# zombie-einstein/bourse

Hardware: NVIDIA B200
Metric: orders_per_sec (higher is better)
Workload: dtype u32

## Files before the change

### bourse_b200/csrc/book.cuh

```cuda
#pragma once
#include <cstdint>

namespace bb {

typedef uint32_t u32;
typedef uint64_t u64;

#define BB_NIL 0xFFFFFFFFu
#define BB_TAG_FREE 0xFFFFFFFFu
#define BB_FULL 0xFFFFFFFFu

enum { ST_NEW = 0, ST_ACTIVE = 1, ST_FILLED = 2, ST_CANCELLED = 3, ST_REJECTED = 4 };
#define META_STATUS_MASK 7u
#define META_BID 8u
#define META_GHOST 16u

#define ERR_CAP_ORDERS 0x01u
#define ERR_CAP_TRADES 0x02u
#define ERR_CAP_PAGES 0x04u
#define ERR_CAP_QUEUE 0x08u
#define ERR_BAD_ID 0x10u
#define ERR_GRANULE 0x20u
#define ERR_CAP_STEPS 0x40u
#define ERR_CAP_LIVE 0x80u
// ... 65 lines not shown
    u32 v;
    asm volatile("ld.global.u32 %0, [%1];" : "=r"(v) : "l"(a));
    return v;
}
__device__ __forceinline__ u64 ldg64(u64 a) {
    u64 v;
    asm volatile("ld.global.u64 %0, [%1];" : "=l"(v) : "l"(a));
    return v;
}
__device__ __forceinline__ uint4 ldg128(u64 a) {
    uint4 v;
    asm volatile("ld.global.v4.u32 {%0,%1,%2,%3}, [%4];" : "=r"(v.x), "=r"(v.y), "=r"(v.z), "=r"(v.w) : "l"(a));
    return v;
}
__device__ __forceinline__ void stg32(u64 a, u32 v) { asm volatile("st.global.u32 [%0], %1;" ::"l"(a), "r"(v) : "memory"); }
__device__ __forceinline__ void stg64(u64 a, u64 v) { asm volatile("st.global.u64 [%0], %1;" ::"l"(a), "l"(v) : "memory"); }
__device__ __forceinline__ void stg128(u64 a, u32 x, u32 y, u32 z, u32 w) {
    asm volatile("st.global.v4.u32 [%0], {%1,%2,%3,%4};" ::"l"(a), "r"(x), "r"(y), "r"(z), "r"(w) : "memory");
}

__device__ __forceinline__ void prefetch_l2(u64 a) { asm volatile("prefetch.global.L2 [%0];" ::"l"(a)); }

#define OH_PRICE 0u
#define OH_VOL 4u
#define OH_NEXT 8u
#define OH_PREV 12u
#define OH_KEYT 16u
#define OH_META 24u
#define OH_SVOL 28u
#define OC_ARR 32u
#define OC_END 40u
#define OC_TRADER 48u
#define PG_VC 0u
#define PG_HT 256u
#define PG_VOL(l) (8u * (l))
#define PG_CNT(l) (8u * (l) + 4u)
#define PG_HEAD(l) (256u + 8u * (l))
#define PG_TAIL(l) (260u + 8u * (l))

#define FL_TRADING 1u
#define FL_HAS_ASK 2u
#define FL_HAS_BID 4u

struct Geo {
    u32 p_total, p_smem, granule, tick, max_orders, max_trades;
    u64 tr_base;
    u64 blobs_base;
    u64 blob_stride;
    u32 d_win_lo, d_levels, d_live;
    u32 pc_off;
};
template <u32 LP_, u32 NWMAX_> struct DenseLayout;
#define ENG_PAGED 0
#define ENG_FAST 1
#define ENG_DENSE 2
#define ENG_DENSE_L 3
#define ENG_PAGED_RES 4
#define ENG_DEEP 5
template <int ENG_> struct GeoT : Geo {
    static constexpr bool FAST = ENG_ == ENG_FAST;
    static constexpr bool RES = ENG_ == ENG_FAST || ENG_ == ENG_PAGED_RES;
    static constexpr bool DENSE = ENG_ == ENG_DENSE || ENG_ == ENG_DENSE_L;
    typedef DenseLayout<(ENG_ == ENG_DENSE_L ? 256u : 128u), (ENG_ == ENG_DENSE_L ? 32u : 8u)> DL;
};
template <class G> __device__ __forceinline__ u32 ptot(const G& g) { return G::FAST ? 32u : g.p_total; }
template <class G> __device__ __forceinline__ u32 gran(const G& g) { return G::FAST ? 1u : g.granule; }

struct Book {
    u64 t, max_key_time;
    u32 n_orders, n_trades, trade_vol;
    u32 vol_ask, vol_bid;
    u32 bq_ask, bq_bid;
    u32 flags, err;
    u32 d_instr, d_trans, d_volume;
    u32 sb;
    u32 tag_lane;
    u64 oh;
    u32 env;
    u64 blob;
    u32 lane;
    u32 free_top;
    u32 ags;
    u64 tr_ptr;
};

__device__ __forceinline__ u32 tag_addr(const Book& b, u32 i) { return b.sb + 128u + 4u * i; }
template <class G> __device__ __forceinline__ u32 vmap_addr(const G& g, const Book& b, u32 i) { return b.sb + 128u + 4u * (ptot(g) + i); }
template <class G> __device__ __forceinline__ u32 qmap_addr(const G& g, const Book& b, u32 i) { return b.sb + 128u + 4u * (2u * ptot(g) + i); }

struct PageS {
    u32 a;
};
struct PageG {
    u64 a;
};
__device__ __forceinline__ u32 pld(PageS p, u32 off) { return lds(p.a + off); }
__device__ __forceinline__ u32 pld(PageG p, u32 off) { return ldg32(p.a + off); }
__device__ __forceinline__ void pst(PageS p, u32 off, u32 v) { sts(p.a + off, v); }
__device__ __forceinline__ void pst(PageG p, u32 off, u32 v) { stg32(p.a + off, v); }
__device__ __forceinline__ uint2 pld2(PageS p, u32 off) {
    const u64 v = lds64(p.a + off);
    return make_uint2((u32)v, (u32)(v >> 32));
}
__device__ __forceinline__ uint2 pld2(PageG p, u32 off) {
    const u64 v = ldg64(p.a + off);
    return make_uint2((u32)v, (u32)(v >> 32));
}
__device__ __forceinline__ void pst2(PageS p, u32 off, u32 x, u32 y) { sts64(p.a + off, ((u64)y << 32) | x); }
__device__ __forceinline__ void pst2(PageG p, u32 off, u32 x, u32 y) { stg64(p.a + off, ((u64)y << 32) | x); }

template <class G> __device__ __forceinline__ u32 page_off(const G& g, u32 slot) { return 128u + 12u * ptot(g) + slot * 512u; }
template <class G> __device__ __forceinline__ PageS page_s(const G& g, const Book& b, u32 slot) {
    return PageS{b.sb + page_off(g, slot)};
}
template <class G> __device__ __forceinline__ PageG page_g(const G& g, const Book& b, u32 slot) {
    return PageG{b.blob + page_off(g, slot)};
}
template <class G> __device__ __forceinline__ uint2 level_pair_any(const G& g, const Book& b, u32 slot, u32 l) {
    return (G::RES || slot < g.p_smem) ? pld2(page_s(g, b, slot), PG_VC + 8u * l) : pld2(page_g(g, b, slot), PG_VC + 8u * l);
}

__device__ __forceinline__ bool has_best(const Book& b, u32 side) { return (b.flags >> (1u + side)) & 1u; }
__device__ __forceinline__ u32 best_q(const Book& b, u32 side) { return side ? b.bq_bid : b.bq_ask; }
__device__ __forceinline__ void set_best(Book& b, u32 side, u32 q) {
    if (side) b.bq_bid = q; else b.bq_ask = q;
    b.flags |= FL_HAS_ASK << side;
}
__device__ __forceinline__ void add_side_vol(Book& b, u32 side, u32 dv) {
    if (side) b.vol_bid += dv; else b.vol_ask += dv;
}

template <class G> __device__ __forceinline__ bool to_level(const G& g, u32 price, u32* q) {
    if (G::FAST || gran(g) == 1u) {
        *q = price;
        return true;
    }
    const u32 x = price / gran(g);
    *q = x;
    return x * gran(g) == price;
}

#define PCACHE_ENTRIES 128u
template <class G> __device__ __forceinline__ u32 find_page(const G& g, const Book& b, u32 side, u32 pkey) {
    const u32 want = (pkey << 1) | side;
    u32 ca = 0;
    if constexpr (!G::FAST) {
        ca = b.sb + g.pc_off + (want & (PCACHE_ENTRIES - 1u));
        const u32 s = lds8(ca);
        if (lds(tag_addr(b, s)) == want) return s;
    }
    for (u32 base = 0; base < ptot(g); base += 32) {
        const u32 m = __ballot_sync(BB_FULL, lds(b.tag_lane + 4u * base) == want);
        if (m) {
            const u32 slot = base + __ffs(m) - 1;
            if constexpr (!G::FAST) sts8(ca, slot);
            return slot;
        }
    }
    return BB_NIL;
}

template <class G> __device__ __forceinline__ u32 alloc_page(const G& g, Book& b, u32 side, u32 pkey) {
    for (u32 base = 0; base < ptot(g); base += 32) {
        const bool usable = !G::RES || (base + b.lane) < g.p_smem;
        const u32 m = __ballot_sync(BB_FULL, usable && lds(b.tag_lane + 4u * base) == BB_TAG_FREE);
        if (m) {
// ... 538 lines not shown
```

### bourse_b200/csrc/dense.cuh

```cuda
#pragma once

namespace bb {

#define D_NIL 0xFFu

template <u32 LP_, u32 NWMAX_> struct DenseLayout {
    static constexpr u32 LP = LP_, NWMAX = NWMAX_;
    static constexpr u32 OFF_ID = 128u, OFF_SV = OFF_ID + 4u * LP, OFF_SL = OFF_SV + 4u * LP, OFF_FS = OFF_SL + 4u * LP;
    static constexpr u32 OFF_BM = OFF_FS + LP, OFF_LV = OFF_BM + 8u * NWMAX;
    static constexpr u32 image_bytes(u32 W) { return OFF_LV + 16u * W; }
};
typedef DenseLayout<128u, 8u> DenseSmall;
typedef DenseLayout<256u, 32u> DenseLarge;

__device__ __forceinline__ void stg128_cs(u64 a, u32 x, u32 y, u32 z, u32 w) {
    asm volatile("st.global.cs.v4.u32 [%0], {%1,%2,%3,%4};" ::"l"(a), "r"(x), "r"(y), "r"(z), "r"(w) : "memory");
}
__device__ __forceinline__ void stg64v(u64 a, u32 x, u32 y) { asm volatile("st.global.v2.u32 [%0], {%1,%2};" ::"l"(a), "r"(x), "r"(y) : "memory"); }

template <class G> __device__ __forceinline__ u32 d_lv(const Book& b, u32 side, u32 q) { return b.sb + G::DL::OFF_LV + 16u * q + 8u * side; }
template <class G> __device__ __forceinline__ u32 d_bm(const Book& b, u32 side, u32 w) {
    return b.sb + G::DL::OFF_BM + 4u * (side ? G::DL::NWMAX : 0u) + 4u * w;
}

template <class G> __device__ __forceinline__ void d_next_best(Book& b, u32 side, u32 q, u32 m) {
    u32 w = q >> 5;
    if (side == 0u) {
        while (m == 0u) {
            if (++w >= G::DL::NWMAX) {
                b.flags &= ~FL_HAS_ASK;
                return;
            }
            m = lds(d_bm<G>(b, 0u, w));
        }
        b.bq_ask = (w << 5) + (u32)__ffs(m) - 1u;
    } else {
        while (m == 0u) {
            if (w == 0u) {
                b.flags &= ~FL_HAS_BID;
                return;
            }
            --w;
            m = lds(d_bm<G>(b, 1u, w));
        }
        b.bq_bid = (w << 5) + 31u - (u32)__clz(m);
    }
}

template <class G> __device__ __forceinline__ void d_log_trade(const G& g, Book& b, u64 t, u32 passive_bid, u32 price, u32 vol,
                                                               u32 active, u32 passive) {
    if (b.n_trades < g.max_trades) {
        stg128_cs(b.tr_ptr, (u32)t, (u32)(t >> 32), price, vol);
        stg128_cs(b.tr_ptr + 16u, active, passive, passive_bid, 0u);
        b.tr_ptr += 32u;
    } else if (g.max_trades) {
        b.err |= ERR_CAP_TRADES;
    }
    b.n_trades += 1;
}

template <class G> __device__ __forceinline__ void d_free_slot(Book& b, u32 slot) {
    sts(b.sb + 4u * slot + G::DL::OFF_ID, BB_NIL);
    sts8(b.sb + G::DL::OFF_FS + b.free_top, slot);
    b.free_top += 1;
}

template <bool STEPPED, class G> __device__ __forceinline__ u32 d_match(const G& g, Book& b, u32 side, u32 price, u32 vol, u32 id, u64 t) {
    const u32 o = side ^ 1u;
    while (vol > 0u && has_best(b, o)) {
        const u32 bq = best_q(b, o);
        const u32 bprice = g.d_win_lo + bq;
        if (side ? (price < bprice) : (price > bprice)) break;
        const u32 la = d_lv<G>(b, o, bq);
        const u64 lv = lds64(la);
        const u32 lvol = (u32)lv, hi = (u32)(lv >> 32);
        const u32 head = (hi >> 16) & 0xFFu;
        const u32 sa = b.sb + 4u * head;
        const u32 pid = lds(sa + G::DL::OFF_ID), pvol = lds(sa + G::DL::OFF_SV);
        const u32 tv = min(vol, pvol);
        vol -= tv;
        d_log_trade(g, b, t, o, bprice, tv, id, pid);
        b.trade_vol += tv;
        if (!STEPPED) {
            b.d_volume += tv;
            b.d_trans += 1;
        }
        add_side_vol(b, o, 0u - tv);
        const u64 pa = b.oh + (u64)pid * ORD_STRIDE;
        if (pvol == tv) {
            stg32(pa + OH_VOL, 0u);
            stg32(pa + OH_META, ST_FILLED | (o ? META_BID : 0u));
            stg64(pa + OC_END, t);
            const u32 nxt = lds8(sa + G::DL::OFF_SL);
            d_free_slot<G>(b, head);
            if ((hi & 0xFFFFu) == 1u) {
                const u32 ba = d_bm<G>(b, o, bq >> 5);
                const u32 m = lds(ba) & ~(1u << (bq & 31u));
                sts(ba, m);
                d_next_best<G>(b, o, bq, m);
            } else {
                sts64(la, ((u64)((hi & 0xFF00FFFFu) - 1u + (nxt << 16)) << 32) | (u64)(lvol - tv));
            }
        } else {
            sts(sa + G::DL::OFF_SV, pvol - tv);
            stg32(pa + OH_VOL, pvol - tv);
            sts(la, lvol - tv);
        }
    }
    return vol;
}

template <bool CHECK_TIME, bool CHECK_SLOTS, class G> __device__ __forceinline__ u32 d_insert(const G& g, Book& b, u32 side, u32 price, u64 t,
                                                                            u32 id, u32 vol) {
    u32 q = price - g.d_win_lo;
    if (q >= g.d_levels) {
        b.err |= ERR_CAP_PAGES;
        q = 0u;
    }
    if (CHECK_SLOTS && b.free_top == 0u) {
        b.err |= ERR_CAP_LIVE;
        return 0u;
    }
    b.free_top -= 1;
    const u32 slot = lds8(b.sb + G::DL::OFF_FS + b.free_top);
    const u32 la = d_lv<G>(b, side, q);
    const u32 ba = d_bm<G>(b, side, q >> 5);
    const u32 bit = 1u << (q & 31u);
    const u32 bw = lds(ba);
    const u32 sa = b.sb + 4u * slot;
    u32 prev = D_NIL;
    if (bw & bit) {
        const u64 lv = lds64(la);
        const u32 hi = (u32)(lv >> 32);
        prev = hi >> 24;
        if (CHECK_TIME && t <= b.max_key_time) {
            const u32 tid = lds(b.sb + 4u * prev + G::DL::OFF_ID);
            if (t <= ldg64(b.oh + (u64)tid * ORD_STRIDE + OH_KEYT)) b.err |= ERR_TIME_ORDER;
        }
        sts64(la, ((u64)(((hi & 0x00FFFFFFu) + 1u) | (slot << 24)) << 32) | (u64)((u32)lv + vol));
        sts8(b.sb + 4u * prev + G::DL::OFF_SL, slot);
    } else {
        sts64(la, ((u64)(1u | (slot << 16) | (slot << 24)) << 32) | (u64)vol);
        sts(ba, bw | bit);
        const bool better = !has_best(b, side) || (side ? q > b.bq_bid : q < b.bq_ask);
        if (better) set_best(b, side, q);
    }
    sts(sa + G::DL::OFF_ID, id);
    sts(sa + G::DL::OFF_SV, vol);
    sts(sa + G::DL::OFF_SL, D_NIL | (prev << 8) | ((q | (side << 15)) << 16));
    add_side_vol(b, side, vol);
    if (CHECK_TIME) {
        if (t > b.max_key_time) b.max_key_time = t;
    } else {
        b.max_key_time = t;
    }
    return slot;
}

template <class G> __device__ __forceinline__ u32 d_find(const Book& b, u32 id) {
#pragma unroll
    for (u32 base = 0; base < G::DL::LP; base += 128u) {
        const uint4 v = lds128(b.sb + G::DL::OFF_ID + 4u * base + 16u * b.lane);
        const u32 hit = v.x == id ? 0u : v.y == id ? 1u : v.z == id ? 2u : v.w == id ? 3u : 4u;
        const u32 m = __ballot_sync(BB_FULL, hit != 4u);
        if (m) {
            const u32 src = (u32)__ffs(m) - 1u;
            return base + 4u * src + __shfl_sync(BB_FULL, hit, src);
        }
    }
    return D_NIL;
}

template <class G> __device__ __forceinline__ void d_remove(Book& b, u32 slot, u32 side, u32 q, u32 next, u32 prev, u32 svol) {
    const u32 la = d_lv<G>(b, side, q);
    const u64 lv = lds64(la);
    const u32 hi = (u32)(lv >> 32);
    if ((hi & 0xFFFFu) == 1u) {
        const u32 ba = d_bm<G>(b, side, q >> 5);
        const u32 m = lds(ba) & ~(1u << (q & 31u));
        sts(ba, m);
        if (best_q(b, side) == q) d_next_best<G>(b, side, q, m);
    } else {
        const u32 head = (hi >> 16) & 0xFFu, tail = hi >> 24;
        const bool is_head = head == slot, is_tail = tail == slot;
        const u32 nh = is_head ? next : head, nt = is_tail ? prev : tail;
        if (!is_head) sts8(b.sb + 4u * prev + G::DL::OFF_SL, next);
        if (!is_tail) sts8(b.sb + 4u * next + G::DL::OFF_SL + 1u, prev);
        sts64(la, ((u64)(((hi & 0xFFFFu) - 1u) | (nh << 16) | (nt << 24)) << 32) | (u64)((u32)lv - svol));
    }
    d_free_slot<G>(b, slot);
    add_side_vol(b, side, 0u - svol);
}

template <bool IS_NEW, bool CHECK_TIME, int HINT, class G>
__device__ __forceinline__ void d_apply(const G& g, Book& b, u32 kind, u32 id, u32 side, u32 price, u32 vol, u32 trader, bool has_p,
                                        bool has_v, u64 t, u32 hint) {
    const u64 ra = b.oh + (u64)id * ORD_STRIDE;
    if (IS_NEW) {
        if (HINT == 0 && id >= g.max_orders) {
            b.err |= ERR_CAP_ORDERS;
            return;
        }
        const bool trading = (b.flags & FL_TRADING) != 0u;
        u32 rem = vol;
        if (trading) rem = d_match<HINT != 0>(g, b, side, price, vol, id, t);
        const bool filled = vol != 0u && rem == 0u;
        const bool market = side ? (price == 0xFFFFFFFFu) : (price == 0u);
        const bool ended = filled || market;
        const u32 status = filled ? ST_FILLED : market ? (trading ? ST_CANCELLED : ST_REJECTED) : ST_ACTIVE;
        if (!ended) {
            const u32 slot = d_insert<CHECK_TIME, HINT == 0>(g, b, side, price, t, id, rem);
            if (HINT == 1 || (HINT == 2 && hint)) sts8(b.ags + hint, slot);
        }
        const u64 kt = ended ? 0ULL : t, end_time = ended ? t : ~0ULL;
        stg64v(ra + OH_PRICE, price, rem);
        stg128(ra + OH_KEYT, (u32)kt, (u32)(kt >> 32), status | (side ? META_BID : 0u), vol);
        stg128(ra + OC_ARR, (u32)t, (u32)(t >> 32), (u32)end_time, (u32)(end_time >> 32));
        stg32(ra + OC_TRADER, trader);
        if (HINT == 0) b.d_trans += 1;
        return;
    }
    if (HINT == 0 && (id >= b.n_orders || id >= g.max_orders)) {
        b.err |= ERR_BAD_ID;
        return;
    }
    u32 slot;
    if (HINT == 1 || (HINT == 2 && hint)) {
        slot = hint - 1u;
        if (lds(b.sb + 4u * slot + G::DL::OFF_ID) != id) return;
    } else {
        slot = d_find<G>(b, id);
        if (slot == D_NIL) return;
    }
    const u32 sa = b.sb + 4u * slot;
    const u32 link = lds(sa + G::DL::OFF_SL), svol = lds(sa + G::DL::OFF_SV);
    const u32 next = link & 0xFFu, prev = (link >> 8) & 0xFFu, q = (link >> 16) & 0x7FFFu;
    side = link >> 31;
    if (kind == EV_MODIFY) {
        if (!has_p && !has_v) return;
        if (!has_p && vol < svol) {
            const u32 la = d_lv<G>(b, side, q);
            sts(sa + G::DL::OFF_SV, vol);
            sts(la, lds(la) - (svol - vol));
            add_side_vol(b, side, vol - svol);
            stg32(ra + OH_VOL, vol);
            b.d_trans += 1;
            return;
        }
        if (!has_p) price = g.d_win_lo + q;
        if (!has_v) vol = svol;
    }
    d_remove<G>(b, slot, side, q, next, prev, svol);
    const u32 side_bit = side ? META_BID : 0u;
    if (kind == EV_CANCEL) {
        stg32(ra + OH_META, ST_CANCELLED | side_bit);
        stg64(ra + OC_END, t);
        b.d_trans += 1;
        return;
    }
    u32 rem = vol;
    if (b.flags & FL_TRADING) rem = d_match<HINT != 0>(g, b, side, price, vol, id, t);
    const bool filled = vol != 0u && rem == 0u;
    if (!filled) d_insert<CHECK_TIME, HINT == 0>(g, b, side, price, t, id, rem);
    stg64v(ra + OH_PRICE, price, rem);
    stg32(ra + OH_META, (filled ? ST_FILLED : ST_ACTIVE) | side_bit);
    stg64(ra + (filled ? OC_END : OH_KEYT), t);
    b.d_trans += 1;
}

template <class G> __device__ __forceinline__ void d_restore(const G& g, Book& b, u32 order_id) {
    const u64 ra = b.oh + (u64)order_id * ORD_STRIDE;
    const uint4 a = ldg128(ra), c = ldg128(ra + 16u);
    if (order_id + 1u > b.n_orders) b.n_orders = order_id + 1u;
    if ((c.z & META_STATUS_MASK) == ST_ACTIVE)
        d_insert<true, true>(g, b, (c.z & META_BID) ? 1u : 0u, a.x, ((u64)c.y << 32) | c.x, order_id, a.y);
}

template <class G> __device__ __forceinline__ void d_level_at(const G& g, const Book& b, u32 side, u32 price, u32* vol, u32* cnt) {
    *vol = 0;
    *cnt = 0;
    const u32 q = price - g.d_win_lo;
    if (q >= g.d_levels) return;
    if (!((lds(d_bm<G>(b, side, q >> 5)) >> (q & 31u)) & 1u)) return;
    const u64 lv = lds64(d_lv<G>(b, side, q));
    *vol = (u32)lv;
    *cnt = (u32)(lv >> 32) & 0xFFFFu;
}

}
```

### bourse_b200/csrc/kernels.cuh

```cuda
#pragma once
#include "../../include/bourse_b200.h"
#include "book.cuh"
#include "philox.cuh"
#include "tma.cuh"
#include "deep.cuh"

namespace bb {

#define MODE_REPLAY 0
#define MODE_ENV 1
#define MAX_GROUPS 8
#define LIVE_CAP 254
#define OBS_STAGE_STEPS(obs_words) ((obs_words) > 9u ? 4u : 8u)

struct MomState {
    double momentum, last_price;
    u32 has_last, n_live;
    u32 live[2];
};
#define MOM_HDR_BYTES 24u
static_assert(sizeof(MomState) == MOM_HDR_BYTES + 8, "MomState layout");

struct KParams {
    unsigned char* blobs;
// ... 298 lines not shown
                        apply_instr<false>(g, b, x.z, x.w, y.x, y.y, y.z, t, false);
                    }
                    __syncwarp();
                }
                b.t = start + p.step_size;
                if (lane == 0u) sts(b.sb + HDR_STEPCTR, lds(b.sb + HDR_STEPCTR) + 1u);
                emit_obs_direct(g, b, p, env);
            }
        }
        if (b.err && lane == 0) atomicOr(p.err_flag, b.err);
        book_to_header(g, b);
        blob_store(p, sb, env, lane);
    }
}

struct Emit {
    u32 n;
    u32 next_id;
};

__device__ __forceinline__ void queue_push(const KParams& p, uint4* q, Emit& e, bool has, u32 op_flags, u32 id, u32 price,
                                           u32 vol, u32 lane) {
    const u32 m = __ballot_sync(BB_FULL, has);
    const u32 pos = e.n + __popc(m & ((1u << lane) - 1u));
    if (has) {
        if (pos < p.max_queue) q[pos] = make_uint4(op_flags, id, price, vol);
    }
    e.n += __popc(m);
}

__device__ __forceinline__ bool order_is_active(const Geo& g, const Book& b, u32 id) {
    return id < g.max_orders && (ldg32(b.oh + (u64)id * ORD_STRIDE + OH_META) & META_STATUS_MASK) == ST_ACTIVE;
}

__device__ __forceinline__ void random_agents_update(const KParams& p, const bb_agent_group& ag, const Book& b, uint4* q,
                                                     Emit& e, u32* slots, u32 env_g, u32 step, u32 slot_base) {
    for (u32 a0 = 0; a0 < ag.n_agents; a0 += 32) {
        const u32 a = a0 + b.lane;
        const bool valid = a < ag.n_agents;
        const uint4 r = philox4x32_10(env_g, step, slot_base + a, 0, p.seed_lo, p.seed_hi);
        const bool active = valid && (u32_to_f32_unit(r.x) < ag.rate);
        u32 held = BB_NIL;
        if (valid) held = slots[slot_base + a];
        bool live = false;
        if (active) live = order_is_active(p.geo, b, held);
        const bool do_cancel = active && live;
        const bool do_new = active && !live;
        const u32 new_mask = __ballot_sync(BB_FULL, do_new);
        const u32 id = e.next_id + __popc(new_mask & ((1u << b.lane) - 1u));
        const u32 side_bid = r.y >> 31;
        const u32 tick = ag.tick_lo + mulhi_range(r.z, ag.tick_hi - ag.tick_lo);
        const u32 vol = ag.vol_lo + mulhi_range(r.w, ag.vol_hi - ag.vol_lo);
        const u32 of = do_cancel ? 0u : (1u | (side_bid << 1) | (a << 13));
        queue_push(p, q, e, active, of, do_cancel ? held : id, tick * ag.tick_size, vol, b.lane);
        e.next_id += __popc(new_mask);
        if (active) slots[slot_base + a] = do_cancel ? BB_NIL : id;
    }
}

template <class G>
__device__ __forceinline__ void random_agents_update_dense(const KParams& p, const bb_agent_group& ag, const Book& b, u32 qs, Emit& e,
                                                           u32 agh, u32 env_g, u32 step, u32 slot_base, u32 chip_base) {
    for (u32 a0 = 0; a0 < ag.n_agents; a0 += 32) {
        const u32 a = a0 + b.lane;
        const bool valid = a < ag.n_agents;
        const u32 ai = valid ? chip_base + a : 0u;
        const uint4 r = philox4x32_10(env_g, step, slot_base + a, 0, p.seed_lo, p.seed_hi);
        const bool active = valid && (u32_to_f32_unit(r.x) < ag.rate);
        const u32 held = lds(agh + 4u * ai);
        const u32 hs = lds8(b.ags + 1u + ai);
        const bool live = held != BB_NIL && lds(b.sb + G::DL::OFF_ID + 4u * hs) == held;
        const bool do_cancel = active && live;
        const bool do_new = active && !live;
        const u32 new_mask = __ballot_sync(BB_FULL, do_new);
        const u32 act_mask = __ballot_sync(BB_FULL, active);
        const u32 below = (1u << b.lane) - 1u;
        const u32 id = e.next_id + __popc(new_mask & below);
        const u32 side_bid = r.y >> 31;
        const u32 tick = ag.tick_lo + mulhi_range(r.z, ag.tick_hi - ag.tick_lo);
        const u32 vol = ag.vol_lo + mulhi_range(r.w, ag.vol_hi - ag.vol_lo);
        const u32 of = do_cancel ? ((hs + 1u) << 2) : (1u | (side_bid << 1) | ((ai + 1u) << 2) | (a << 13));
        const u32 pos = e.n + __popc(act_mask & below);
        if (active) {
            if (pos < p.max_queue) sts128(qs + 16u * pos, make_uint4(of, do_cancel ? held : id, tick * ag.tick_size, vol));
            sts(agh + 4u * ai, do_cancel ? BB_NIL : id);
        }
        e.n += __popc(act_mask);
        e.next_id += __popc(new_mask);
    }
}

__device__ __forceinline__ u32 warp_excl_scan(u32 v, u32 lane, u32* total) {
    u32 x = v;
#pragma unroll
    for (int d = 1; d < 32; d <<= 1) {
        const u32 y = __shfl_up_sync(BB_FULL, x, d);
        if (lane >= (u32)d) x += y;
    }
    *total = __shfl_sync(BB_FULL, x, 31);
    return x - v;
}

__device__ __forceinline__ u32 round_price(double x, double tick, bool up) {
    x = (up ? ceil(x / tick) : floor(x / tick)) * tick;
    x = fmin(fmax(x, 0.0), 4294967295.0);
    return (u32)x;
}

struct MomOut {
    u32 n, next_id, err;
};
__device__ __noinline__ MomOut momentum_agent_update(const KParams& p, const bb_agent_group& ag, u64 oh, u32 lane, u32 bid,
                                                     u32 ask, uint4* q, u32 e_n, u32 e_next_id, MomState* ms, u32 env_g,
                                                     u32 step, u32 gi, u32 slot_base) {
    Emit e;
    e.n = e_n;
    e.next_id = e_next_id;
    u32 err = 0;
    const u32 n_live = ms->n_live;
    u32 n_keep = 0;
    for (u32 k0 = 0; k0 < n_live; k0 += 32) {
        const u32 k = k0 + lane;
        const bool valid = k < n_live;
        u32 id = BB_NIL;
        bool active = false;
        if (valid) {
            id = ms->live[k];
            active = id < p.geo.max_orders && (ldg32(oh + (u64)id * ORD_STRIDE + OH_META) & META_STATUS_MASK) == ST_ACTIVE;
        }
        const uint4 r = philox4x32_10(env_g, step, PHILOX_SLOT_CANCEL | gi, k >> 2, p.seed_lo, p.seed_hi);
        const u32 word = (k & 3u) == 0 ? r.x : (k & 3u) == 1 ? r.y : (k & 3u) == 2 ? r.z : r.w;
        const bool keep = active && (u32_to_f32_unit(word) > ag.rate);
        const bool cancel = active && !keep;
        queue_push(p, q, e, cancel, 0u, id, 0, 0, lane);
        const u32 km = __ballot_sync(BB_FULL, keep);
        __syncwarp();
        if (keep) ms->live[n_keep + __popc(km & ((1u << lane) - 1u))] = id;
        n_keep += __popc(km);
        __syncwarp();
    }
    const double mid = (double)bid + 0.5 * (double)(u32)(ask - bid);
    const bool noise = ag.kind == BB_GROUP_NOISE;
    double m = 0.0, p_market = 0.0;
    if (!noise && ms->has_last) {
        m = ms->momentum * (1.0 - ag.decay) + ag.decay * (mid - ms->last_price);
        p_market = ag.demand * tanh(ag.scale * m) / (double)ag.n_agents;
    }
    const double p_limit = ag.order_ratio * p_market;
    const double tick = (double)ag.tick_size;
    for (u32 j0 = 0; j0 < ag.n_agents; j0 += 32) {
        const u32 j = j0 + lane;
        const bool valid = j < ag.n_agents;
        const uint4 ra = philox4x32_10(env_g, step, slot_base + j, 0, p.seed_lo, p.seed_hi);
        const uint4 rb = philox4x32_10(env_g, step, slot_base + j, 1, p.seed_lo, p.seed_hi);
        const bool dir = (m > 0.0) || (m < 0.0);
        bool do_limit = valid && dir && (u64_to_f64_unit(ra.x, ra.y) < p_limit);
        bool do_market = valid && dir && (u64_to_f64_unit(ra.z, ra.w) < p_market);
        bool limit_bid = m > 0.0, market_bid = m > 0.0;
        if (noise) {
            do_limit = valid && (u32_to_f32_unit(ra.x) < (float)ag.decay);
            limit_bid = (ra.y >> 31) != 0;
            do_market = valid && (u32_to_f32_unit(ra.z) < (float)ag.demand);
            market_bid = (ra.w >> 31) != 0;
        }
        u32 price = 0;
        if (do_limit) {
            double u1 = u64_to_f64_unit(rb.x, rb.y);
// ... 202 lines not shown
                }
            }
            __syncwarp();

            const u64 start = b.t;
            b.trade_vol = 0;
            if constexpr (G::DENSE) {
                if (n > p.step_size || (start <= b.max_key_time && (b.flags & (FL_HAS_ASK | FL_HAS_BID)))) b.err |= ERR_TIME_ORDER;
            }
            u32 nq = n, mk_off = 0, mk_loc = 0, mk_all = 0;
            if constexpr (MKT) {
                const u32 cb = mk_sb + 4u * MAX_GROUPS * (mk_phase & 1u);
                mk_phase += 1;
                const bool own = lane < p.n_groups && p.group_asset[lane] == mk_a;
                if (own) sts(cb + 4u * lane, mk_cnt);
                market_bar_sync(mk_bar, 32u * p.assets);
                mk_all = lane < p.n_groups ? lds(cb + 4u * lane) : 0u;
                u32 total, total_mine;
                mk_off = warp_excl_scan(mk_all, lane, &total);
                mk_loc = warp_excl_scan(own ? mk_all : 0u, lane, &total_mine);
                nq = total;
                if (nq > p.assets * p.max_queue) {
                    b.err |= ERR_CAP_QUEUE;
                    nq = 0;
                }
                if constexpr (G::DENSE) {
                    if (nq > p.step_size) b.err |= ERR_TIME_ORDER;
                }
            }
            if constexpr (MKT || !G::DENSE)
                for (u32 i = lane; i < nq; i += 32) sts16(perm + 2u * i, i);
            for (u32 b0 = 0; b0 * 4u < nq; b0 += 32) {
                const u32 blk = b0 + lane;
                if (blk * 4u < nq) {
                    const uint4 r = philox4x32_10(env_g, step, PHILOX_SLOT_SHUFFLE, blk, p.seed_lo, p.seed_hi);
                    const u32 i = blk * 4u;
                    const u32 j0 = mulhi_range(r.x, i + 1), j1 = mulhi_range(r.y, i + 2);
                    const u32 j2 = mulhi_range(r.z, i + 3), j3 = mulhi_range(r.w, i + 4);
                    sts(jarr + 2u * i, j0 | (j1 << 16));
                    sts(jarr + 2u * i + 4u, j2 | (j3 << 16));
                }
            }
            __syncwarp();
            if (lane != 0u) {
            } else if constexpr (G::DENSE && !MKT) {
                for (u32 i = n; i > 1; --i) {
                    const u32 j = lds16(jarr + 2u * (i - 1));
                    const uint4 x = lds128(qs + 16u * (i - 1)), y = lds128(qs + 16u * j);
                    sts128(qs + 16u * (i - 1), y);
                    sts128(qs + 16u * j, x);
                }
            } else {
                for (u32 i = nq; i > 1; --i) {
                    const u32 j = lds16(jarr + 2u * (i - 1));
                    const u32 x = lds16(perm + 2u * (i - 1)), y = lds16(perm + 2u * j);
                    sts16(perm + 2u * (i - 1), y);
                    sts16(perm + 2u * j, x);
                }
            }
            __syncwarp();
            if constexpr (MKT) {
                u32 n_mine = 0;
                for (u32 i0 = 0; i0 < nq; i0 += 32) {
                    const u32 i = i0 + lane;
                    const u32 gq = i < nq ? lds16(perm + 2u * i) : 0xFFFFFFFFu;
                    bool is_mine = false;
                    u32 li = 0;
                    for (u32 k = 0; k < p.n_groups; ++k) {
                        const u32 o = __shfl_sync(BB_FULL, mk_off, k), c = __shfl_sync(BB_FULL, mk_all, k);
                        const u32 lo = __shfl_sync(BB_FULL, mk_loc, k);
                        if (gq - o < c && p.group_asset[k] == mk_a) {
                            is_mine = true;
                            li = lo + (gq - o);
                        }
                    }
                    const u32 m = __ballot_sync(BB_FULL, is_mine);
                    const u32 pos = n_mine + __popc(m & ((1u << lane) - 1u));
                    if (is_mine && pos < p.max_queue) sts(jarr + 4u * pos, min(li, p.max_queue - 1u) | (i << 16));
                    n_mine += __popc(m);
                }
                n = min(n, n_mine);
                __syncwarp();
            }
            if constexpr (G::DENSE) {
                constexpr int H = MOM ? 2 : 1;
                const u32 nt0 = b.n_trades;
                if (MOM || lane == 0) {
                    auto handle = [&](const uint4& ev) {
                        const u32 hint = (ev.x >> 2) & 0x7FFu;
                        if (ev.x & 1u) {
                            if (ev.x & 2u) book_apply<true, false, G, H>(g, b, EV_NEW, ev.y, 1u, ev.z, ev.w, ev.x >> 13, false, false, b.t, hint);
                            else book_apply<true, false, G, H>(g, b, EV_NEW, ev.y, 0u, ev.z, ev.w, ev.x >> 13, false, false, b.t, hint);
                        } else {
                            book_apply<false, false, G, H>(g, b, EV_CANCEL, ev.y, 0u, 0u, 0u, 0u, false, false, b.t, hint);
                        }
                        b.t += 1;
                    };
                    if constexpr (MKT) {
                        for (u32 k = 0; k < n; ++k) {
                            const u32 w = lds(jarr + 4u * k);
                            const uint4 ev = lds128(qs + 16u * (w & 0xFFFFu));
                            b.t = start + (u64)(w >> 16);
                            handle(ev);
                        }
                    } else {
                    uint4 e0 = lds128(qs);
                    for (u32 i = 0; i < n; i += 2) {
                        const uint4 e1 = lds128(qs + 16u * i + 16u);
                        handle(e0);
                        if (i + 1 >= n) break;
                        e0 = lds128(qs + 16u * i + 32u);
                        handle(e1);
                    }
                    }
                }
                if constexpr (!MOM) {
                    __syncwarp();
                    b.max_key_time = __shfl_sync(BB_FULL, b.max_key_time, 0);
                    b.n_trades = __shfl_sync(BB_FULL, b.n_trades, 0);
                    b.trade_vol = __shfl_sync(BB_FULL, b.trade_vol, 0);
                    b.vol_ask = __shfl_sync(BB_FULL, b.vol_ask, 0);
                    b.vol_bid = __shfl_sync(BB_FULL, b.vol_bid, 0);
                    b.bq_ask = __shfl_sync(BB_FULL, b.bq_ask, 0);
                    b.bq_bid = __shfl_sync(BB_FULL, b.bq_bid, 0);
                    b.flags = __shfl_sync(BB_FULL, b.flags, 0);
                    b.err = __shfl_sync(BB_FULL, b.err, 0);
                    b.d_trans = __shfl_sync(BB_FULL, b.d_trans, 0);
                    b.d_volume = __shfl_sync(BB_FULL, b.d_volume, 0);
                    b.free_top = __shfl_sync(BB_FULL, b.free_top, 0);
                    b.tr_ptr = __shfl_sync(BB_FULL, b.tr_ptr, 0);
                }
                b.d_trans += (b.n_trades - nt0) + (n ? e.next_id - id0 : 0u);
                b.d_volume += b.trade_vol;
            } else
            for (u32 i0 = 0; i0 < n; i0 += 32) {
                const u32 cnt = min(32u, n - i0);
                uint4 mine = make_uint4(0, 0, 0, 0);
                u32 toff = 0;
                if (lane < cnt) {
                    if constexpr (MKT) {
                        const u32 w = lds(jarr + 4u * (i0 + lane));
                        mine = ldg128(qa + 16u * (w & 0xFFFFu));
                        toff = w >> 16;
                    } else {
                        mine = ldg128(qa + 16u * lds16(perm + 2u * (i0 + lane)));
                    }
                }
                for (u32 k = 0; k < cnt; ++k) {
                    if constexpr (MKT) b.t = start + (u64)__shfl_sync(BB_FULL, toff, k);
                    const u32 of = __shfl_sync(BB_FULL, mine.x, k), id = __shfl_sync(BB_FULL, mine.y, k);
                    const u32 price = __shfl_sync(BB_FULL, mine.z, k), vol = __shfl_sync(BB_FULL, mine.w, k);
                    if (of & 1u) {
                        if constexpr (MOM) book_apply<true, false>(g, b, EV_NEW, id, (of >> 1) & 1u, price, vol, of >> 13, false, false, b.t);
                        else if (of & 2u) book_apply<true, false>(g, b, EV_NEW, id, 1u, price, vol, of >> 13, false, false, b.t);
                        else book_apply<true, false>(g, b, EV_NEW, id, 0u, price, vol, of >> 13, false, false, b.t);
                    } else {
                        book_apply<false, false>(g, b, EV_CANCEL, id, 0u, 0u, 0u, 0u, false, false, b.t);
                    }
                    b.t += 1;
                }
            }
            b.d_instr += n;
            b.t = start + p.step_size;
            __syncwarp();

            if (staged) {
                u32 w0, w1;
// ... 591 lines not shown
```

Baseline: 5.541 billion.

## Journal dense-book matching in shared memory and flush global writes warp-parallel

```diff
diff --git a/bourse_b200/csrc/book.cuh b/bourse_b200/csrc/book.cuh
--- a/bourse_b200/csrc/book.cuh
+++ b/bourse_b200/csrc/book.cuh
@@ -171,6 +171,7 @@
     u32 free_top;
     u32 ags;
     u64 tr_ptr;
+    u32 ev, jp, jend;
 };
 
 __device__ __forceinline__ u32 tag_addr(const Book& b, u32 i) { return b.sb + 128u + 4u * i; }
diff --git a/bourse_b200/csrc/dense.cuh b/bourse_b200/csrc/dense.cuh
--- a/bourse_b200/csrc/dense.cuh
+++ b/bourse_b200/csrc/dense.cuh
@@ -65,12 +65,13 @@
     b.free_top += 1;
 }
 
-template <bool STEPPED, class G> __device__ __forceinline__ u32 d_match(const G& g, Book& b, u32 side, u32 price, u32 vol, u32 id, u64 t) {
+template <bool STEPPED, bool JRN, class G> __device__ __forceinline__ u32 d_match(const G& g, Book& b, u32 side, u32 price, u32 vol, u32 id, u64 t) {
     const u32 o = side ^ 1u;
     while (vol > 0u && has_best(b, o)) {
         const u32 bq = best_q(b, o);
         const u32 bprice = g.d_win_lo + bq;
         if (side ? (price < bprice) : (price > bprice)) break;
+        if (JRN && b.jp == b.jend) break;
         const u32 la = d_lv<G>(b, o, bq);
         const u64 lv = lds64(la);
         const u32 lvol = (u32)lv, hi = (u32)(lv >> 32);
@@ -79,8 +80,13 @@
         const u32 pid = lds(sa + G::DL::OFF_ID), pvol = lds(sa + G::DL::OFF_SV);
         const u32 tv = min(vol, pvol);
         vol -= tv;
-        d_log_trade(g, b, t, o, bprice, tv, id, pid);
-        b.trade_vol += tv;
+        if (JRN) {
+            sts128(b.jp, make_uint4(b.ev | (bq << 20), pid, tv, pvol - tv));
+            b.jp += 16u;
+        } else {
+            d_log_trade(g, b, t, o, bprice, tv, id, pid);
+            b.trade_vol += tv;
+        }
         if (!STEPPED) {
             b.d_volume += tv;
             b.d_trans += 1;
@@ -88,9 +94,11 @@
         add_side_vol(b, o, 0u - tv);
         const u64 pa = b.oh + (u64)pid * ORD_STRIDE;
         if (pvol == tv) {
-            stg32(pa + OH_VOL, 0u);
-            stg32(pa + OH_META, ST_FILLED | (o ? META_BID : 0u));
-            stg64(pa + OC_END, t);
+            if (!JRN) {
+                stg32(pa + OH_VOL, 0u);
+                stg32(pa + OH_META, ST_FILLED | (o ? META_BID : 0u));
+                stg64(pa + OC_END, t);
+            }
             const u32 nxt = lds8(sa + G::DL::OFF_SL);
             d_free_slot<G>(b, head);
             if ((hi & 0xFFFFu) == 1u) {
@@ -103,15 +111,15 @@
             }
         } else {
             sts(sa + G::DL::OFF_SV, pvol - tv);
-            stg32(pa + OH_VOL, pvol - tv);
+            if (!JRN) stg32(pa + OH_VOL, pvol - tv);
             sts(la, lvol - tv);
         }
     }
     return vol;
 }
 
-template <bool CHECK_TIME, bool CHECK_SLOTS, class G> __device__ __forceinline__ u32 d_insert(const G& g, Book& b, u32 side, u32 price, u64 t,
-                                                                            u32 id, u32 vol) {
+template <bool CHECK_TIME, bool CHECK_SLOTS, bool JRN, class G>
+__device__ __forceinline__ u32 d_insert(const G& g, Book& b, u32 side, u32 price, u64 t, u32 id, u32 vol) {
     u32 q = price - g.d_win_lo;
     if (q >= g.d_levels) {
         b.err |= ERR_CAP_PAGES;
@@ -151,7 +159,7 @@
     add_side_vol(b, side, vol);
     if (CHECK_TIME) {
         if (t > b.max_key_time) b.max_key_time = t;
-    } else {
+    } else if (!JRN) {
         b.max_key_time = t;
     }
     return slot;
@@ -192,25 +200,31 @@
     add_side_vol(b, side, 0u - svol);
 }
 
-template <bool IS_NEW, bool CHECK_TIME, int HINT, class G>
-__device__ __forceinline__ void d_apply(const G& g, Book& b, u32 kind, u32 id, u32 side, u32 price, u32 vol, u32 trader, bool has_p,
-                                        bool has_v, u64 t, u32 hint) {
+template <bool IS_NEW, bool CHECK_TIME, int HINT, bool JRN = false, class G>
+__device__ __forceinline__ u32 d_apply(const G& g, Book& b, u32 kind, u32 id, u32 side, u32 price, u32 vol, u32 trader, bool has_p,
+                                       bool has_v, u64 t, u32 hint) {
+    static_assert(!JRN || HINT == 1, "the journal derives order ids from the agents' hints");
     const u64 ra = b.oh + (u64)id * ORD_STRIDE;
     if (IS_NEW) {
         if (HINT == 0 && id >= g.max_orders) {
             b.err |= ERR_CAP_ORDERS;
-            return;
+            return 0u;
         }
         const bool trading = (b.flags & FL_TRADING) != 0u;
         u32 rem = vol;
-        if (trading) rem = d_match<HINT != 0>(g, b, side, price, vol, id, t);
+        if (trading) rem = d_match<HINT != 0, JRN>(g, b, side, price, vol, id, t);
+        if (JRN && rem != 0u && b.jp == b.jend) return rem;
         const bool filled = vol != 0u && rem == 0u;
         const bool market = side ? (price == 0xFFFFFFFFu) : (price == 0u);
         const bool ended = filled || market;
         const u32 status = filled ? ST_FILLED : market ? (trading ? ST_CANCELLED : ST_REJECTED) : ST_ACTIVE;
         if (!ended) {
-            const u32 slot = d_insert<CHECK_TIME, HINT == 0>(g, b, side, price, t, id, rem);
+            const u32 slot = d_insert<CHECK_TIME, HINT == 0, JRN>(g, b, side, price, t, id, rem);
             if (HINT == 1 || (HINT == 2 && hint)) sts8(b.ags + hint, slot);
+        }
+        if (JRN) {
+            sts(b.ev + 4u, rem);
+            return 0u;
         }
         const u64 kt = ended ? 0ULL : t, end_time = ended ? t : ~0ULL;
         stg64v(ra + OH_PRICE, price, rem);
@@ -218,26 +232,26 @@
         stg128(ra + OC_ARR, (u32)t, (u32)(t >> 32), (u32)end_time, (u32)(end_time >> 32));
         stg32(ra + OC_TRADER, trader);
         if (HINT == 0) b.d_trans += 1;
-        return;
+        return 0u;
     }
     if (HINT == 0 && (id >= b.n_orders || id >= g.max_orders)) {
         b.err |= ERR_BAD_ID;
-        return;
+        return 0u;
     }
     u32 slot;
     if (HINT == 1 || (HINT == 2 && hint)) {
         slot = hint - 1u;
-        if (lds(b.sb + 4u * slot + G::DL::OFF_ID) != id) return;
+        if (lds(b.sb + 4u * slot + G::DL::OFF_ID) != id) return 0u;
     } else {
         slot = d_find<G>(b, id);
-        if (slot == D_NIL) return;
+        if (slot == D_NIL) return 0u;
     }
     const u32 sa = b.sb + 4u * slot;
     const u32 link = lds(sa + G::DL::OFF_SL), svol = lds(sa + G::DL::OFF_SV);
     const u32 next = link & 0xFFu, prev = (link >> 8) & 0xFFu, q = (link >> 16) & 0x7FFFu;
     side = link >> 31;
     if (kind == EV_MODIFY) {
-        if (!has_p && !has_v) return;
+        if (!has_p && !has_v) return 0u;
         if (!has_p && vol < svol) {
             const u32 la = d_lv<G>(b, side, q);
             sts(sa + G::DL::OFF_SV, vol);
@@ -245,27 +259,101 @@
             add_side_vol(b, side, vol - svol);
             stg32(ra + OH_VOL, vol);
             b.d_trans += 1;
-            return;
+            return 0u;
         }
         if (!has_p) price = g.d_win_lo + q;
         if (!has_v) vol = svol;
     }
     d_remove<G>(b, slot, side, q, next, prev, svol);
     const u32 side_bit = side ? META_BID : 0u;
-    if (kind == EV_CANCEL) {
-        stg32(ra + OH_META, ST_CANCELLED | side_bit);
-        stg64(ra + OC_END, t);
+    if (JRN || kind == EV_CANCEL) {
+        if (JRN) {
+            sts(b.ev + 12u, 2u | side);
+        } else {
+            stg32(ra + OH_META, ST_CANCELLED | side_bit);
+            stg64(ra + OC_END, t);
+        }
         b.d_trans += 1;
-        return;
+        return 0u;
     }
     u32 rem = vol;
-    if (b.flags & FL_TRADING) rem = d_match<HINT != 0>(g, b, side, price, vol, id, t);
+    if (b.flags & FL_TRADING) rem = d_match<HINT != 0, false>(g, b, side, price, vol, id, t);
     const bool filled = vol != 0u && rem == 0u;
-    if (!filled) d_insert<CHECK_TIME, HINT == 0>(g, b, side, price, t, id, rem);
+    if (!filled) d_insert<CHECK_TIME, HINT == 0, false>(g, b, side, price, t, id, rem);
     stg64v(ra + OH_PRICE, price, rem);
     stg32(ra + OH_META, (filled ? ST_FILLED : ST_ACTIVE) | side_bit);
     stg64(ra + (filled ? OC_END : OH_KEYT), t);
     b.d_trans += 1;
+    return 0u;
+}
+
+template <class G>
+__device__ __forceinline__ void d_flush(const G& g, Book& b, u32 qs, u32 agh, u64 start, u32 e_lo, u32 e_hi, u32 jb, u32 nj) {
+    const bool trading = (b.flags & FL_TRADING) != 0u;
+    u32 last_rest = 0;
+    for (u32 i = e_lo + b.lane; i < e_hi; i += 32u) {
+        const uint4 ev = lds128(qs + 16u * i);
+        const u64 t = start + i;
+        const u32 side_bit = (ev.x & 2u) ? META_BID : 0u;
+        if (ev.x & 1u) {
+            const u32 id = lds(agh + 4u * ((ev.x >> 2) & 0x7FFu) - 4u);
+            const u32 price = ev.z, vol = ev.w, rem = ev.y;
+            const bool filled = vol != 0u && rem == 0u;
+            const bool market = side_bit ? (price == 0xFFFFFFFFu) : (price == 0u);
+            const bool ended = filled || market;
+            const u32 status = filled ? ST_FILLED : market ? (trading ? ST_CANCELLED : ST_REJECTED) : ST_ACTIVE;
+            if (!ended) last_rest = i + 1u;
+            const u64 ra = b.oh + (u64)id * ORD_STRIDE;
+            const u64 kt = ended ? 0ULL : t, end_time = ended ? t : ~0ULL;
+            stg64v(ra + OH_PRICE, price, rem);
+            stg128(ra + OH_KEYT, (u32)kt, (u32)(kt >> 32), status | side_bit, vol);
+            stg128(ra + OC_ARR, (u32)t, (u32)(t >> 32), (u32)end_time, (u32)(end_time >> 32));
+            stg32(ra + OC_TRADER, ev.x >> 13);
+        } else if (ev.w) {
+            const u64 ra = b.oh + (u64)ev.y * ORD_STRIDE;
+            stg32(ra + OH_META, ST_CANCELLED | ((ev.w & 1u) ? META_BID : 0u));
+            stg64(ra + OC_END, t);
+        }
+    }
+    last_rest = __reduce_max_sync(BB_FULL, last_rest);
+    if (last_rest) b.max_key_time = start + (last_rest - 1u);
+    __syncwarp();
+    u32 err = 0, tv_sum = 0;
+    const u64 tr_env = g.tr_base + (u64)b.env * g.max_trades * 32u;
+    for (u32 k0 = 0; k0 < nj; k0 += 32u) {
+        const u32 k = k0 + b.lane;
+        const bool valid = k < nj;
+        const uint4 je = valid ? lds128(jb + 16u * k) : make_uint4(0u, BB_NIL, 0u, 0u);
+        const u32 same = __match_any_sync(BB_FULL, je.y);
+        if (valid) {
+            const u32 ea = je.x & 0xFFFFFu, pid = je.y, tv = je.z, left = je.w;
+            const u32 ax = lds(ea);
+            const u32 active = lds(agh + 4u * ((ax >> 2) & 0x7FFu) - 4u);
+            const u32 o = ((ax >> 1) & 1u) ^ 1u;
+            const u64 t = start + ((ea - qs) >> 4);
+            const u32 idx = b.n_trades + k;
+            if (idx < g.max_trades) {
+                const u64 ta = tr_env + (u64)idx * 32u;
+                stg128_cs(ta, (u32)t, (u32)(t >> 32), g.d_win_lo + (je.x >> 20), tv);
+                stg128_cs(ta + 16u, active, pid, o, 0u);
+            } else if (g.max_trades) {
+                err |= ERR_CAP_TRADES;
+            }
+            if ((same >> b.lane) == 1u) {
+                const u64 pa = b.oh + (u64)pid * ORD_STRIDE;
+                stg32(pa + OH_VOL, left);
+                if (left == 0u) {
+                    stg32(pa + OH_META, ST_FILLED | (o ? META_BID : 0u));
+                    stg64(pa + OC_END, t);
+                }
+            }
+            tv_sum += tv;
+        }
+        __syncwarp();
+    }
+    b.trade_vol += __reduce_add_sync(BB_FULL, tv_sum);
+    b.n_trades += nj;
+    b.err |= __reduce_or_sync(BB_FULL, err);
 }
 
 template <class G> __device__ __forceinline__ void d_restore(const G& g, Book& b, u32 order_id) {
@@ -273,7 +361,7 @@
     const uint4 a = ldg128(ra), c = ldg128(ra + 16u);
     if (order_id + 1u > b.n_orders) b.n_orders = order_id + 1u;
     if ((c.z & META_STATUS_MASK) == ST_ACTIVE)
-        d_insert<true, true>(g, b, (c.z & META_BID) ? 1u : 0u, a.x, ((u64)c.y << 32) | c.x, order_id, a.y);
+        d_insert<true, true, false>(g, b, (c.z & META_BID) ? 1u : 0u, a.x, ((u64)c.y << 32) | c.x, order_id, a.y);
 }
 
 template <class G> __device__ __forceinline__ void d_level_at(const G& g, const Book& b, u32 side, u32 price, u32* vol, u32* cnt) {
diff --git a/bourse_b200/csrc/kernels.cuh b/bourse_b200/csrc/kernels.cuh
--- a/bourse_b200/csrc/kernels.cuh
+++ b/bourse_b200/csrc/kernels.cuh
@@ -404,7 +404,7 @@
         const u32 of = do_cancel ? ((hs + 1u) << 2) : (1u | (side_bid << 1) | ((ai + 1u) << 2) | (a << 13));
         const u32 pos = e.n + __popc(act_mask & below);
         if (active) {
-            if (pos < p.max_queue) sts128(qs + 16u * pos, make_uint4(of, do_cancel ? held : id, tick * ag.tick_size, vol));
+            if (pos < p.max_queue) sts128(qs + 16u * pos, make_uint4(of, do_cancel ? held : id, tick * ag.tick_size, do_cancel ? 0u : vol));
             sts(agh + 4u * ai, do_cancel ? BB_NIL : id);
         }
         e.n += __popc(act_mask);
@@ -773,7 +773,59 @@
                 n = min(n, n_mine);
                 __syncwarp();
             }
-            if constexpr (G::DENSE) {
+            if constexpr (G::DENSE && !MOM && !MKT) {
+                const u32 nt0 = b.n_trades;
+                const u32 jb = qs + 16u * n, jend = qs + 16u * (p.max_queue + 2u);
+                u32 done = 0, rv = 0;
+                for (;;) {
+                    u32 stop = n;
+                    if (lane == 0) {
+                        b.jp = jb;
+                        b.jend = jend;
+                        auto handle = [&](const uint4& ev, u32 i) -> u32 {
+                            const u32 hint = (ev.x >> 2) & 0x7FFu;
+                            b.ev = qs + 16u * i;
+                            if (ev.x & 1u) {
+                                if (ev.x & 2u) return d_apply<true, false, 1, true>(g, b, EV_NEW, ev.y, 1u, ev.z, ev.w, 0u, false, false, 0ull, hint);
+                                return d_apply<true, false, 1, true>(g, b, EV_NEW, ev.y, 0u, ev.z, ev.w, 0u, false, false, 0ull, hint);
+                            }
+                            return d_apply<false, false, 1, true>(g, b, EV_CANCEL, ev.y, 0u, 0u, 0u, 0u, false, false, 0ull, hint);
+                        };
+                        uint4 e0 = lds128(qs + 16u * done);
+                        if (rv) e0.w = rv;
+                        for (u32 i = done; i < n; i += 2) {
+                            const uint4 e1 = lds128(qs + 16u * i + 16u);
+                            if ((rv = handle(e0, i))) {
+                                stop = i;
+                                break;
+                            }
+                            if (i + 1 >= n) break;
+                            e0 = lds128(qs + 16u * i + 32u);
+                            if ((rv = handle(e1, i + 1))) {
+                                stop = i + 1;
+                                break;
+                            }
+                        }
+                    }
+                    __syncwarp();
+                    stop = __shfl_sync(BB_FULL, stop, 0);
+                    rv = __shfl_sync(BB_FULL, rv, 0);
+                    const u32 nj = (__shfl_sync(BB_FULL, b.jp, 0) - jb) >> 4;
+                    b.vol_ask = __shfl_sync(BB_FULL, b.vol_ask, 0);
+                    b.vol_bid = __shfl_sync(BB_FULL, b.vol_bid, 0);
+                    b.bq_ask = __shfl_sync(BB_FULL, b.bq_ask, 0);
+                    b.bq_bid = __shfl_sync(BB_FULL, b.bq_bid, 0);
+                    b.flags = __shfl_sync(BB_FULL, b.flags, 0);
+                    b.d_trans = __shfl_sync(BB_FULL, b.d_trans, 0);
+                    b.free_top = __shfl_sync(BB_FULL, b.free_top, 0);
+                    b.err = __shfl_sync(BB_FULL, b.err, 0);
+                    d_flush(g, b, qs, agh, start, done, stop, jb, nj);
+                    done = stop;
+                    if (stop == n) break;
+                }
+                b.d_trans += (b.n_trades - nt0) + (n ? e.next_id - id0 : 0u);
+                b.d_volume += b.trade_vol;
+            } else if constexpr (G::DENSE) {
                 constexpr int H = MOM ? 2 : 1;
                 const u32 nt0 = b.n_trades;
                 if (MOM || lane == 0) {
```

Measured after the change: 6.286 billion (median of 6 runs). 1.13x the previous value.
